# zongh5a/MDF-Net

Measured on AMD Instinct MI355X. Metric: views/sec at DTU 1600x1200x5-view x4-scale, higher is better.
Workload: dtype f32; 1 GPU; DTU eval 1600x1184 (1600x1200 cropped as load/dtueval.py:34), 5 views, 3 cost-volume stages + x2 refine = 4 output scales, hypotheses (48,24,8), batch 1 per rank, seeded random weights (pth/dtu_29.pth is not available offline); parallelism=views sharded over 1 rank(s), no collective

## Files before the change

### mdf-net_amd/csrc/conv_lds.hip

```cpp
#include <cstdlib>
#include <mutex>
#include <type_traits>
#include "common.h"

#include "conv_lds_common.h"

namespace {

constexpr int kSchedSlots = 128;
__device__ unsigned g_sched[2 * kSchedSlots];
#ifdef MDF_STAMPS
__device__ unsigned long long g_stamps[8];
#define STAMP() __builtin_readcyclecounter()
#endif

template <typename C, int KD, int KHW, int SHW, int COUT, int MTL, int ST = 0>
__device__ __forceinline__ void step(const float* const (&planes)[KD], __amdgpu_buffer_rsrc_t wres, int wvoff, const LdsConvParams& p,
                                     size_t row_vox, int w0, int q, int n16, const float (&wr)[C::WN][C::NT][C::KPL],
                                     const float (&al)[C::NT][4], const float (&be)[C::NT][4], const float (&wfirst)[2][C::NT][C::KPL]) {
  constexpr int NT = C::NT;
  extern __shared__ __attribute__((aligned(16))) float lds_base_[];
  const float* epi_tab = lds_base_ + C::EPI_OFF;
  static_assert(ST == 0 || COUT % 4 == 0, "epilogue sums need Cout % 4 == 0");
  f32x4 acc[MTL][NT];
// ... 681 lines not shown
    long long ipb = C::STREAM ? 2 : ((C::RD == 2 && blocks_per_cu == 1) ? 3 : 6);
    if (const char* e = getenv("MDF_CONV_ITEMS_PER_BLOCK")) { if (atoi(e) > 0) ipb = atoi(e); }
    long long want = (ipb * max_grid + tiles - 1) / tiles;
    if (want < 1) want = 1;
    if (want > p.D / 3) want = p.D / 3;
    if (want < 1) want = 1;
    int dch = (int)((p.D + want - 1) / want);
    if (C::RD == 2 && (dch & 1)) ++dch;
    {
      const long long items0 = tiles * ((p.D + dch - 1) / dch);
      if (items0 > max_grid && items0 < 3 * (long long)max_grid) {
        const long long rounds0 = (items0 + max_grid - 1) / max_grid;
        for (int d2 = dch + C::RD; d2 <= p.D + C::RD - 1; d2 += C::RD) {
          if (tiles * ((p.D + d2 - 1) / d2) <= max_grid) {
            if (10 * (d2 + C::NPL - 1) < 9 * rounds0 * (dch + C::NPL - 1)) dch = d2;
            break;
          }
        }
      }
    }
    if (const char* e = getenv("MDF_CONV_DCH")) { if (atoi(e) > 0) dch = atoi(e); }
    if (C::RD == 2 && (dch & 1)) ++dch;
    p.dch = dch;
    p.dchunks = (p.D + dch - 1) / dch;
    const long long items = tiles * p.dchunks;
    if (items > 0x7fffffff) return mdf::fail(MDF_EARG, "conv_lds: too many work items");
    p.n_items = (int)items;
  } else {
    if (p.D != 1) return mdf::fail(MDF_EARG, "2-D conv path needs D == 1");
    if (tiles > 0x7fffffff) return mdf::fail(MDF_EARG, "conv_lds: too many tiles");
    p.n_tiles = (int)tiles;
    p.tiles_per_item = 0;
    long long tpb = 2;
    if (const char* e = getenv("MDF_CONV2D_TILES_PER_BLOCK")) { if (atoi(e) > 0) tpb = atoi(e); }
    long long g = tiles / tpb;
    if (g < 256) g = 256;
    if (g > max_grid) g = max_grid;
    if (g > tiles) g = tiles;
    p.n_items = (int)g;
    p.dch = 1; p.dchunks = 1;
  }
  static bool attr_done_dev[64] = {};
  int dev_id = 0;
  (void)hipGetDevice(&dev_id);
  bool& attr_done = attr_done_dev[(dev_id >= 0 && dev_id < 64) ? dev_id : 0];
  if (!attr_done || dev_id >= 64) {
    hipError_t e = hipFuncSetAttribute(reinterpret_cast<const void*>(&conv_lds_kernel<CIN, CIN_MEM, COUT, KD, KHW, SHW, MT, RW, WG, ST>),
                                       hipFuncAttributeMaxDynamicSharedMemorySize, (int)kLds);
    if (e != hipSuccess) return mdf::fail(MDF_EHIP, "hipFuncSetAttribute(dynamic LDS %zu): %s", kLds, hipGetErrorString(e));
    attr_done = true;
  }
  int grid = max_grid;
  if (const char* g = getenv("MDF_CONV_GRID")) { if (atoi(g) > 0) grid = atoi(g); }
  if (grid > p.n_items) grid = p.n_items;
  if (ST) {
    if (KD == 1) {
      const int G = p.stat_groups > 0 ? p.stat_groups : 1;
      int bpg = grid / G;
      if (bpg < 1) bpg = 1;
      grid = G * bpg;
      p.stat_slices = mdf::conv_stat_slices(bpg, p.stat_slices);
    } else {
      p.stat_slices = mdf::conv_stat_slices(grid, p.stat_slices);
    }
  }
  if (getenv("MDF_CONV_DEBUG")) {
    int nb = -1;
    hipError_t e = hipOccupancyMaxActiveBlocksPerMultiprocessor(&nb, conv_lds_kernel<CIN, CIN_MEM, COUT, KD, KHW, SHW, MT, RW, WG, ST>, 256, kLds);
    hipFuncAttributes fa{};
    (void)hipFuncGetAttributes(&fa, reinterpret_cast<const void*>(&conv_lds_kernel<CIN, CIN_MEM, COUT, KD, KHW, SHW, MT, RW, WG, ST>));
    fprintf(stderr, "[conv_lds<%d,%d,%d,%d,%d,%d,%d,rw%d>] LDS %zu B dyn + %zu static, regs %d, occupancy API: %d blocks/CU (%s), grid %d, items %d\n",
            CIN, CIN_MEM, COUT, KD, KHW, SHW, MT, RW, kLds, fa.sharedSizeBytes, fa.numRegs, nb, hipGetErrorString(e), grid, p.n_items);
  }
  hipLaunchKernelGGL((conv_lds_kernel<CIN, CIN_MEM, COUT, KD, KHW, SHW, MT, RW, WG, ST>), dim3(grid), dim3(256), kLds, st, p);
  return mdf::check_launch("conv_lds_kernel");
}

}

#ifdef MDF_STAMPS
extern "C" int mdf_debug_read_stamps(unsigned long long* out8, int reset) {
  hipError_t e = hipMemcpyFromSymbol(out8, HIP_SYMBOL(g_stamps), sizeof(unsigned long long) * 8);
  if (e != hipSuccess) return -3;
  if (reset) {
    unsigned long long z[8] = {0};
    (void)hipMemcpyToSymbol(HIP_SYMBOL(g_stamps), z, sizeof z);
  }
  return 0;
}
#endif

#define LDS_CASE(ci, cim, co, kd, k, s, mt)                                                      \
  if (!stat && Cin == ci && Cin_mem == cim && Cout == co && KD == kd && KHW == k && stride == s) \
    return launch_lds<ci, cim, co, kd, k, s, mt>(p, (hipStream_t)stream);
#define LDS_CASE_T(ci, cim, co, kd, k, s, mt)                                                    \
  if (Cin == ci && Cin_mem == cim && Cout == co && KD == kd && KHW == k && stride == s)          \
    return !stat ? launch_lds<ci, cim, co, kd, k, s, mt>(p, (hipStream_t)stream) : (stat->mode == 1 ? launch_lds<ci, cim, co, kd, k, s, mt, 1, 0, 1>(p, (hipStream_t)stream) : launch_lds<ci, cim, co, kd, k, s, mt, 1, 0, 2>(p, (hipStream_t)stream));

namespace {
std::mutex g_slot_mu;
void* g_slot_stream[kSchedSlots];
bool g_slot_used[kSchedSlots];
}

static int sched_slot_of(void* stream) {
  std::lock_guard<std::mutex> lock(g_slot_mu);
  int free_slot = -1;
  for (int i = 0; i < kSchedSlots; ++i) {
    if (g_slot_used[i] && g_slot_stream[i] == stream) return i;
    if (!g_slot_used[i] && free_slot < 0) free_slot = i;
  }
  if (free_slot >= 0) { g_slot_used[free_slot] = true; g_slot_stream[free_slot] = stream; }
  return free_slot;
}

extern "C" int mdf_release_stream(void* stream) {
  std::lock_guard<std::mutex> lock(g_slot_mu);
  for (int i = 0; i < kSchedSlots; ++i)
    if (g_slot_used[i] && g_slot_stream[i] == stream) { g_slot_used[i] = false; g_slot_stream[i] = nullptr; return MDF_OK; }
  return MDF_OK;
}

#define LDS_CASE_RW(ci, cim, co, kd, k, s, mt, rw)                                               \
  if (!stat && use_rw && Cin == ci && Cin_mem == cim && Cout == co && KD == kd && KHW == k && stride == s && !res_up) { \
    p.wpack = wpack + (size_t)kd * k * k * ci * 16;                                              \
    return launch_lds<ci, cim, co, kd, k, s, mt, rw>(p, (hipStream_t)stream);                    \
  }
#define LDS_CASE_RW_T(ci, cim, co, kd, k, s, mt, rw)                                             \
  if (use_rw && Cin == ci && Cin_mem == cim && Cout == co && KD == kd && KHW == k && stride == s && !res_up) { \
    p.wpack = wpack + (size_t)kd * k * k * ci * 16;                                              \
    return !stat ? launch_lds<ci, cim, co, kd, k, s, mt, rw>(p, (hipStream_t)stream) : (stat->mode == 1 ? launch_lds<ci, cim, co, kd, k, s, mt, rw, 0, 1>(p, (hipStream_t)stream) : launch_lds<ci, cim, co, kd, k, s, mt, rw, 0, 2>(p, (hipStream_t)stream)); \
  }

#define LDS_CASE_WG(ci, co)                                                                      \
  if (use_wg && KD == 3 && KHW == 3 && stride == 1 && Cin == ci && Cin_mem == ci && Cout == co && !res_up) { \
    p.wpack = wpack + (size_t)27 * ci * (((co + 15) / 16) * 16) + (co == 8 ? (size_t)36 * ci * 16 : 0); \
    return !stat ? launch_lds<ci, ci, co, 3, 3, 1, 1, 2, 1>(p, (hipStream_t)stream) : (stat->mode == 1 ? launch_lds<ci, ci, co, 3, 3, 1, 1, 2, 1, 1>(p, (hipStream_t)stream) : launch_lds<ci, ci, co, 3, 3, 1, 1, 2, 1, 2>(p, (hipStream_t)stream)); \
  }
#define LDS_CASE_WG2(ci, co)                                                                     \
  if (use_wg && KD == 1 && KHW == 3 && stride == 1 && Cin == ci && Cin_mem == ci && Cout == co && !res_up && (!shuffle2 || (ci == 16 && co == 32) || (ci == 32 && co == 64))) { \
    p.wpack = wpack + (size_t)9 * ci * (((co + 15) / 16) * 16);                                  \
    return !stat ? launch_lds<ci, ci, co, 1, 3, 1, 1, 2, 1>(p, (hipStream_t)stream) : (stat->mode == 1 ? launch_lds<ci, ci, co, 1, 3, 1, 1, 2, 1, 1>(p, (hipStream_t)stream) : launch_lds<ci, ci, co, 1, 3, 1, 1, 2, 1, 2>(p, (hipStream_t)stream)); \
  }

#define LDS_CASE_WD(ci)                                                                          \
  if (use_wd && KD == 3 && KHW == 3 && stride == 1 && Cin == ci && Cin_mem == ci && Cout == 8 && !res_up && D >= 2) { \
    p.wpack = wpack + (size_t)27 * ci * 16 + (size_t)36 * ci * 16 + (ci == 16 ? (size_t)3 * 16 * 64 * 4 : 0); \
    if (ci == 16 && wd_stream && !stat) return launch_lds<ci, ci, 8, 3, 3, 1, 1, 2, 3>(p, (hipStream_t)stream); \
    return !stat ? launch_lds<ci, ci, 8, 3, 3, 1, 1, 2, 2>(p, (hipStream_t)stream) : (stat->mode == 1 ? launch_lds<ci, ci, 8, 3, 3, 1, 1, 2, 2, 1>(p, (hipStream_t)stream) : launch_lds<ci, ci, 8, 3, 3, 1, 1, 2, 2, 2>(p, (hipStream_t)stream)); \
  }

int mdf_wino3d_dispatch(const float* x, const float* wpack_wino, const float* alpha, const float* beta, const float* res, float res_scale,
                        float* y, int B, int D, int H, int W, int Cin, int Cout, int relu, void* stream);
int mdf_wino2d_dispatch(const float* x, const float* wpack_wino, const float* alpha, const float* beta, const float* res, float res_scale,
                        float* y, int B, int H, int W, int Cin, int Cout, int relu, void* stream);
int mdf_wino2d_s2d_dispatch(const float* x, const float* wpack_k5w, const float* alpha, const float* beta, float* y, int B, int Ho, int Wo,
                            int Cin_mem, int Cout, int relu, void* stream);

int mdf_conv_lds_dispatch(const float* x, const float* wpack, const float* alpha, const float* beta, const float* res,
                          float res_scale, const float* res_up, float* y, int B, int D, int H, int W, int Cin, int Cin_mem, int Cout, int KD,
                          int KHW, int stride, int relu, void* stream, int planar_in, int shuffle2, const mdf::ConvStat* stat) {
  static const int wd_mask = [] { const char* e = getenv("MDF_CONV_WD"); return e ? atoi(e) : 3; }();
  const bool wd_stream = [] { const char* e = getenv("MDF_CONV_WD_STREAM"); return e ? atoi(e) != 0 : true; }();
  static const bool use_wg = [] { const char* e = getenv("MDF_CONV_WINOGRAD"); return e ? atoi(e) != 0 : true; }();
  static const bool use_rw = [] { const char* e = getenv("MDF_CONV_RW"); return e ? atoi(e) != 0 : true; }();
  LdsConvParams p{};
  p.x = x; p.wpack = wpack; p.alpha = alpha; p.beta = beta; p.res = res; p.res_scale = res_scale; p.res_up = res_up; p.y = y;
  p.B = B; p.D = D; p.H = H; p.W = W; p.relu = relu; p.planar_in = planar_in; p.shuffle2 = shuffle2;
  if (stat) {
    if (Cout % 4 != 0 || shuffle2 || res_up) return mdf::fail(MDF_EUNSUPPORTED, "epilogue sums: Cout %% 4 == 0, no pixel-shuffle / upsample-add");
    p.stat_mode = stat->mode; p.stat_y = stat->y; p.stat_aux = stat->aux; p.stat_out = stat->out; p.stat_slices = stat->nslices;
    p.stat_groups = (KD == 1 && stat->group_imgs > 0) ? B / stat->group_imgs : 1;
  }
  p.sched_slot = sched_slot_of(stream);
  if (p.sched_slot < 0) return mdf::fail(MDF_EUNSUPPORTED, "conv kernels support up to %d distinct HIP streams per process", kSchedSlots);
  {
    const char* e = getenv("MDF_CONV_PREFETCH_EARLY");
    p.prefetch_early = e ? atoi(e) : 0;
  }
  const int pad = (KHW - 1) / 2;
  p.Ho = (H + 2 * pad - KHW) / stride + 1;
  p.Wo = (W + 2 * pad - KHW) / stride + 1;
  {
    const bool k5w = [] { const char* e = getenv("MDF_CONV_K5_WINOGRAD"); return e ? atoi(e) != 0 : true; }();
    if (use_wg && k5w && KD == 1 && KHW == 5 && stride == 2 && !stat && !res_up && !shuffle2 && !planar_in && H % 2 == 0 && W % 2 == 0) {
      const bool use_w2 = [] { const char* e = getenv("MDF_CONV_WINO2D"); return e ? atoi(e) != 0 : true; }();
      if (use_w2 && !res && Cin == Cin_mem && ((Cin == 16 && Cout == 32) || (Cin == 8 && Cout == 16))) {
        const size_t plain = (size_t)25 * 64 * (Cin == 16 ? 2 * 4 : 1 * 2);
        const int rc = mdf_wino2d_s2d_dispatch(x, wpack + plain, alpha, beta, y, B, p.Ho, p.Wo, Cin, Cout, relu, stream);
        if (rc != MDF_EUNSUPPORTED) return rc;
      }
      if (Cin == 16 && Cin_mem == 16 && Cout == 32) {
        p.s2d = 1; p.wpack = wpack + (size_t)25 * 1 * 2 * 64 * 4;
        return launch_lds<64, 64, 32, 1, 3, 1, 1, 2, 1>(p, (hipStream_t)stream);
      }
    }
  }
  if (shuffle2 && Cout == 64 && !use_wg) return mdf::fail(MDF_EUNSUPPORTED, "pixel-shuffle store for Cout = 64 is built into the Winograd form only (MDF_CONV_WINOGRAD=0 is set)");
  { const bool use_wd = use_wg && (wd_mask & 1); LDS_CASE_WD(8) }
  { const bool use_wd = use_wg && (wd_mask & 2); LDS_CASE_WD(16) }
  {
    const bool use_w3 = [] { const char* e = getenv("MDF_CONV_WINO3D"); return e ? atoi(e) != 0 : true; }();
    if (use_wg && use_w3 && !stat && KD == 3 && KHW == 3 && stride == 1 && Cin == Cin_mem && !res_up && !shuffle2 && Cout % 16 == 0) {
      const int rc = mdf_wino3d_dispatch(x, wpack + (size_t)27 * Cin * Cout, alpha, beta, res, res_scale, y, B, D, H, W, Cin, Cout, relu, stream);
      if (rc != MDF_EUNSUPPORTED) return rc;
    }
  }
  {
    const bool use_w2 = [] { const char* e = getenv("MDF_CONV_WINO2D"); return e ? atoi(e) != 0 : true; }();
    if (use_wg && use_w2 && !stat && KD == 1 && KHW == 3 && stride == 1 && Cin == Cin_mem && !res_up && !shuffle2 && !planar_in && D == 1) {
      const int rc = mdf_wino2d_dispatch(x, wpack + (size_t)9 * Cin * (((Cout + 15) / 16) * 16), alpha, beta, res, res_scale, y, B, H, W, Cin, Cout, relu, stream);
      if (rc != MDF_EUNSUPPORTED) return rc;
    }
  }
  LDS_CASE_WG(16, 16) LDS_CASE_WG(32, 16) LDS_CASE_WG(32, 32) LDS_CASE_WG(16, 8) LDS_CASE_WG(16, 32)
  LDS_CASE_WG2(16, 16) LDS_CASE_WG2(32, 32) LDS_CASE_WG2(64, 64) LDS_CASE_WG2(16, 32) LDS_CASE_WG2(32, 64)
  LDS_CASE_RW_T(16, 16, 8, 3, 3, 1, 2, 2) LDS_CASE_RW_T(8, 8, 8, 3, 3, 1, 2, 2)
  LDS_CASE_RW(16, 16, 4, 1, 3, 1, 1, 4) LDS_CASE_RW(8, 8, 4, 1, 3, 1, 1, 4)
  LDS_CASE_RW_T(8, 8, 8, 1, 3, 1, 2, 2) LDS_CASE_RW_T(4, 3, 8, 1, 3, 1, 2, 2) LDS_CASE_RW(4, 1, 8, 1, 3, 1, 2, 2)
  LDS_CASE(32, 32, 16, 3, 3, 1, 2) LDS_CASE(16, 16, 16, 3, 3, 1, 4) LDS_CASE(16, 16, 8, 3, 3, 1, 4) LDS_CASE(8, 8, 8, 3, 3, 1, 4)
  LDS_CASE(32, 32, 32, 3, 3, 1, 2)
  LDS_CASE(16, 16, 32, 3, 3, 1, 2) LDS_CASE(8, 8, 16, 3, 3, 1, 4)
  LDS_CASE(4, 3, 8, 1, 3, 1, 4) LDS_CASE(8, 8, 8, 1, 3, 1, 4) LDS_CASE(16, 16, 16, 1, 3, 1, 4) LDS_CASE(32, 32, 32, 1, 3, 1, 2)
  LDS_CASE(64, 64, 64, 1, 3, 1, 1)
  LDS_CASE_T(8, 8, 16, 1, 5, 2, 2) LDS_CASE_T(16, 16, 32, 1, 5, 2, 2) LDS_CASE_T(32, 32, 64, 1, 5, 2, 1)
  LDS_CASE(16, 16, 32, 1, 1, 1, 4)
  LDS_CASE(16, 16, 64, 1, 1, 1, 4) LDS_CASE(32, 32, 64, 1, 1, 1, 2) LDS_CASE(64, 64, 16, 1, 1, 1, 1) LDS_CASE(64, 64, 32, 1, 1, 1, 1)
  LDS_CASE(64, 64, 64, 1, 1, 1, 1)
  LDS_CASE(32, 32, 32, 1, 1, 1, 2) LDS_CASE(32, 32, 16, 1, 1, 1, 2) LDS_CASE(16, 16, 16, 1, 1, 1, 4)
  LDS_CASE(4, 1, 8, 1, 3, 1, 4) LDS_CASE(8, 8, 32, 1, 3, 1, 4) LDS_CASE(8, 8, 1, 1, 3, 1, 4)
  LDS_CASE(32, 32, 8, 1, 3, 1, 2)
  LDS_CASE(16, 16, 32, 1, 3, 1, 2) LDS_CASE(32, 32, 64, 1, 3, 1, 1)
  LDS_CASE(16, 16, 4, 1, 3, 1, 4) LDS_CASE(8, 8, 4, 1, 3, 1, 4)
  return MDF_EUNSUPPORTED;
}
```

### mdf-net_amd/csrc/wino3d.hip

```cpp
#include <cstdlib>
#include <type_traits>
#include "common.h"
#include "conv_lds_common.h"
#include "wino3d_acc.h"

namespace {

template <int I, int N, typename F>
__device__ __forceinline__ void static_for(F&& f) {
  if constexpr (I < N) {
    f(std::integral_constant<int, I>{});
    static_for<I + 1, N>(f);
  }
}

struct Wino3dParams {
  const float* x;
  const float* wpack;
  const float* alpha;
  const float* beta;
  const float* res;
  float* y;
  float res_scale;
  int B, D, H, W, relu;
// ... 207 lines not shown
          float ov[4];
#pragma unroll
          for (int k = 0; k < 4; ++k) {
            ov[k] = yv[pr][rr][k] * al_l[k] + be_l[k];
            if (p.relu) ov[k] = fmaxf(ov[k], 0.f);
          }
          const size_t oi = (row_vox + ow) * COUT + c0;
          if (p.res) {
            const float4 rv = *reinterpret_cast<const float4*>(p.res + oi);
            ov[0] = rv.x + ov[0] * p.res_scale; ov[1] = rv.y + ov[1] * p.res_scale;
            ov[2] = rv.z + ov[2] * p.res_scale; ov[3] = rv.w + ov[3] * p.res_scale;
          }
          if (!(MDF_W3_DIAG & 2) || ov[0] == 1234.5f) *reinterpret_cast<float4*>(p.y + oi) = make_float4(ov[0], ov[1], ov[2], ov[3]);
        }
      }
    };

    auto step = [&](auto rc, int zi, int z_next2, bool has_next, bool k0, bool k1, bool k2, bool fresh1) {
      constexpr int R = decltype(rc)::value;
      const bool all3 = MDF_W3_NOMASK || (k0 && k1 && k2 && !fresh1);
      if (MDF_W3_PF_AT_START) issue_plane(has_next ? zi + 1 : -1);
      constexpr int SLOT_N = (R + 1) % 3;
      static_for<0, NSTEP>([&](auto ic) {
        constexpr int i = decltype(ic)::value;
        constexpr int ch = i / 16, ab = i % 16;
        constexpr bool last_chunk = (ch == NCH - 1);
        if (!(MDF_W3_DIAG & 16)) load_a((i + AH) % NSTEP, (i + AH) % NA);
        if constexpr (ch == 0 && ab == WRITE_AB) {
          if (has_next) {
            write_plane(SLOT_N);
            __syncthreads();
          }
        }
        if constexpr (ab > WRITE_AB && ab <= WRITE_AB + 8) {
          constexpr int e0 = 2 * (ab - WRITE_AB - 1);
          if constexpr (!last_chunk) { read_elem(R, ch + 1, e0); read_elem(R, ch + 1, e0 + 1); }
          else { read_elem(SLOT_N, 0, e0); read_elem(SLOT_N, 0, e0 + 1); }
        }
        __builtin_amdgcn_sched_barrier(0);
        constexpr int S0 = ((R + 1) % 3) * 16 + ab, S1 = R * 16 + ab, S2 = ((R + 2) % 3) * 16 + ab;
        if (__builtin_expect(all3, 1)) {
          if constexpr (ch == 0) AccTile<S0>::mfma_fresh(af[i % NA][0][0], V[ab][0][0]);
          else AccTile<S0>::mfma(af[i % NA][0][0], V[ab][0][0]);
          AccTile<S0>::mfma(af[i % NA][0][1], V[ab][0][1]);
          AccTile<S0>::mfma(af[i % NA][0][2], V[ab][1][0]);
          AccTile<S0>::mfma(af[i % NA][0][3], V[ab][1][1]);
          AccTile<S1>::mfma(af[i % NA][1][0], V[ab][0][0]);
          AccTile<S1>::mfma(af[i % NA][1][1], V[ab][0][1]);
          AccTile<S1>::mfma(af[i % NA][1][2], V[ab][1][0]);
          AccTile<S1>::mfma(af[i % NA][1][3], V[ab][1][1]);
          AccTile<S2>::mfma(af[i % NA][2][0], V[ab][0][0]);
          AccTile<S2>::mfma(af[i % NA][2][1], V[ab][0][1]);
          AccTile<S2>::mfma(af[i % NA][2][2], V[ab][1][0]);
          AccTile<S2>::mfma(af[i % NA][2][3], V[ab][1][1]);
        } else {
          if (k0) {
            if constexpr (ch == 0) AccTile<S0>::mfma_fresh(af[i % NA][0][0], V[ab][0][0]);
            else AccTile<S0>::mfma(af[i % NA][0][0], V[ab][0][0]);
            AccTile<S0>::mfma(af[i % NA][0][1], V[ab][0][1]);
            AccTile<S0>::mfma(af[i % NA][0][2], V[ab][1][0]);
            AccTile<S0>::mfma(af[i % NA][0][3], V[ab][1][1]);
          }
          if (k1) {
            if constexpr (ch == 0) {
              if (fresh1) AccTile<S1>::mfma_fresh(af[i % NA][1][0], V[ab][0][0]);
              else AccTile<S1>::mfma(af[i % NA][1][0], V[ab][0][0]);
            } else {
              AccTile<S1>::mfma(af[i % NA][1][0], V[ab][0][0]);
            }
            AccTile<S1>::mfma(af[i % NA][1][1], V[ab][0][1]);
            AccTile<S1>::mfma(af[i % NA][1][2], V[ab][1][0]);
            AccTile<S1>::mfma(af[i % NA][1][3], V[ab][1][1]);
          }
          if (k2) {
            AccTile<S2>::mfma(af[i % NA][2][0], V[ab][0][0]);
            AccTile<S2>::mfma(af[i % NA][2][1], V[ab][0][1]);
            AccTile<S2>::mfma(af[i % NA][2][2], V[ab][1][0]);
            AccTile<S2>::mfma(af[i % NA][2][3], V[ab][1][1]);
          }
        }
        __builtin_amdgcn_sched_barrier(0);
        if constexpr (ab == 15 && !last_chunk) { if (!(MDF_W3_DIAG & 8)) transform(); }
      });
      if (!MDF_W3_PF_AT_START) issue_plane(z_next2);
      if (!(MDF_W3_DIAG & 8)) transform();
      if (k2 && !(MDF_W3_DIAG & 4)) epilogue(std::integral_constant<int, (R + 2) % 3>{}, zi - 1);
    };

    int zi = (da == 0) ? 0 : da - 1;
    const int z_last = (db == p.D) ? p.D - 1 : db;
    __syncthreads();
    issue_plane(zi);
    write_plane(0);
    __syncthreads();
    if (!MDF_W3_PF_AT_START) issue_plane(zi < z_last ? zi + 1 : -1);
#pragma unroll
    for (int e = 0; e < 16; ++e) read_elem(0, 0, e);
    transform();
#pragma unroll
    for (int i = 0; i < AH; ++i) load_a(i, i % NA);

    int r_last = 0;
#define W3_STEP(RR)                                                                                          \
    {                                                                                                        \
      const bool has_next = zi < z_last;                                                                     \
      step(std::integral_constant<int, RR>{}, zi, (zi + 2 <= z_last) ? zi + 2 : -1, has_next,                \
           zi + 1 >= da && zi + 1 < db, zi >= da && zi < db, zi - 1 >= da && zi - 1 < db, zi == 0);          \
      if (!has_next) { r_last = RR; break; }                                                                 \
      ++zi;                                                                                                  \
    }
    for (;;) {
      W3_STEP(0)
      W3_STEP(1)
      W3_STEP(2)
    }
#undef W3_STEP
    if (db == p.D) {
      switch (r_last) {
        case 0: epilogue(std::integral_constant<int, 0>{}, p.D - 1); break;
        case 1: epilogue(std::integral_constant<int, 1>{}, p.D - 1); break;
        default: epilogue(std::integral_constant<int, 2>{}, p.D - 1); break;
      }
    }
  }
}

template <int CIN, int COUT>
int launch_wino3d(Wino3dParams& p, hipStream_t st) {
  typedef W3<CIN, COUT> C;
  constexpr int NA = MDF_W3_NA;
  constexpr int WRITE_AB = MDF_W3_WRITE_AB;
  p.tiles_h = (p.H + C::TH - 1) / C::TH;
  p.tiles_w = (p.W + C::TWO - 1) / C::TWO;
  p.total = (long long)p.B * p.tiles_h * p.tiles_w * p.D;
  if (p.total >= (1ll << 31)) return MDF_EUNSUPPORTED;
  auto kern = &wino3d_kernel<CIN, COUT, NA, WRITE_AB>;
  static bool attr_done_dev[64] = {};
  int dev_id = 0;
  (void)hipGetDevice(&dev_id);
  bool& attr_done = attr_done_dev[(dev_id >= 0 && dev_id < 64) ? dev_id : 0];
  if (!attr_done || dev_id >= 64) {
    hipError_t e = hipFuncSetAttribute(reinterpret_cast<const void*>(kern), hipFuncAttributeMaxDynamicSharedMemorySize, (int)C::LDS_BYTES);
    if (e != hipSuccess) return mdf::fail(MDF_EHIP, "hipFuncSetAttribute(dynamic LDS %zu): %s", (size_t)C::LDS_BYTES, hipGetErrorString(e));
    attr_done = true;
  }
  long long grid = 256;
  if (const char* g = getenv("MDF_WINO3D_GRID")) { if (atoi(g) > 0) grid = atoi(g); }
  if (grid > p.total / 4) grid = p.total / 4;
  if (grid < 1) grid = 1;
  hipLaunchKernelGGL(kern, dim3((unsigned)grid), dim3(256), C::LDS_BYTES, st, p);
  return mdf::check_launch("wino3d_kernel");
}

}

int mdf_wino3d_dispatch(const float* x, const float* wpack_wino, const float* alpha, const float* beta, const float* res, float res_scale,
                        float* y, int B, int D, int H, int W, int Cin, int Cout, int relu, void* stream) {
  Wino3dParams p{};
  p.x = x; p.wpack = wpack_wino; p.alpha = alpha; p.beta = beta; p.res = res; p.res_scale = res_scale; p.y = y;
  p.B = B; p.D = D; p.H = H; p.W = W; p.relu = relu;
  if ((long long)H * W * Cin * 4 >= (1ll << 31)) return MDF_EUNSUPPORTED;
  if (Cin == 32 && Cout == 16) return launch_wino3d<32, 16>(p, (hipStream_t)stream);
  if (Cin == 16 && Cout == 16) return launch_wino3d<16, 16>(p, (hipStream_t)stream);
  return MDF_EUNSUPPORTED;
}
```

### mdf-net_amd/mdfnet_hip/kernel_families.py

```python
import re

MFMA_CONV = "mfma_conv"
WARP = "warp_aggregate"
WARP_TRAIN = "aggregate_train_passes"
WARP_SCATTER = "aggregate_scatter"
WGRAD = "wgrad"
BN = "batchnorm_train"
PROB = "prob_head"
HEADS = "heads"
FILTER = "consistency_filter"
POINT_EVAL = "point_eval"
CONTROL = "control"

KERNEL_FAMILY = {
    "conv_lds_kernel": MFMA_CONV, "conv3d_kernel": MFMA_CONV, "conv3d_wlds_kernel": MFMA_CONV, "convtr_all_kernel": MFMA_CONV, "convtr_cls_kernel": MFMA_CONV, "conv_pair_kernel": MFMA_CONV, "conv_pair_valu_kernel": MFMA_CONV,
    "conv1x1_kernel": MFMA_CONV, "conv1x1_heads_kernel": MFMA_CONV, "refine_tail_kernel": MFMA_CONV, "prob_fused_kernel": MFMA_CONV, "res_pair_kernel": MFMA_CONV,
    "wino3d_kernel": MFMA_CONV, "wino2d_kernel": MFMA_CONV,
    "pack_weights_kernel": CONTROL, "pack_batch_kernel": CONTROL,
    "warp_kernel": WARP, "warp_vec8_kernel": WARP, "warp_vec_win_kernel": WARP, "corner_index_kernel": WARP,
    "warp_train_kernel": WARP_TRAIN, "warp_bwd_kernel": WARP_SCATTER,
    "agg_prepare_kernel": CONTROL, "agg_finalize_kernel": CONTROL, "agg_bwd_finalize_kernel": WARP_SCATTER,
    "wgrad_kernel": WGRAD, "wgrad_a1_kernel": WGRAD, "wgrad_a1_valu_kernel": WGRAD, "wgrad2d_kernel": WGRAD,
    "wgrad_lds_kernel": WGRAD, "wgrad_lds_batch_kernel": WGRAD, "slab_sum_kernel": WGRAD, "slab_sum_batch_kernel": WGRAD,
    "bn_reduce_kernel": BN, "bn_finalize_kernel": BN, "bn_relu_apply_kernel": BN, "bn_finalize_apply_kernel": BN,
    "bn_relu_bwd_kernel": BN,
    "prob_head_kernel": PROB, "prob_head_tiled_kernel": PROB, "prob_from_partials_kernel": PROB,
    "softmax_regress_bwd_kernel": PROB, "prob_conv_dgrad_kernel": PROB, "upsample2_bwd_kernel": PROB,
    "depth_regress_kernel": HEADS, "confidence_kernel": HEADS, "confidence_up2_kernel": HEADS, "range_affine_kernel": HEADS,
    "hypos_fit_kernel": HEADS, "hypos_from_fit_kernel": HEADS, "refine_head_kernel": HEADS, "fpn_compose_fwd_kernel": HEADS, "fpn_compose_bwd_kernel": HEADS,
    "consistency_fuse_kernel": FILTER,
    "consensus_fuse_kernel": FILTER, "consensus_scan_kernel": FILTER, "consensus_compact_kernel": FILTER,
    "pcd_reproj_kernel": FILTER, "pcd_cand_count_kernel": FILTER, "pcd_cand_place_kernel": FILTER, "pcd_select_kernel": FILTER, "pcd_select_big_kernel": FILTER, "pcd_bin_sum_kernel": FILTER, "pcd_bin_offsets_kernel": FILTER,
    "pcd_seg_init_kernel": FILTER, "pcd_seg_hook_kernel": FILTER, "pcd_seg_count_kernel": FILTER, "pcd_seg_apply_kernel": FILTER,
    "pcd_count_kernel": FILTER, "pcd_scan_kernel": FILTER, "pcd_compact_kernel": FILTER,
    "pts_bbox_kernel": POINT_EVAL, "pts_bbox_final_kernel": POINT_EVAL, "pts_morton_kernel": POINT_EVAL, "pts_sort_hist_kernel": POINT_EVAL,
    "pts_sort_scan_kernel": POINT_EVAL, "pts_sort_scatter_kernel": POINT_EVAL, "pts_gather_kernel": POINT_EVAL, "pts_leaf_kernel": POINT_EVAL,
    "pts_node_kernel": POINT_EVAL, "pts_nn_kernel": POINT_EVAL, "pts_rank_kernel": POINT_EVAL, "pts_radius_kernel": POINT_EVAL,
    "pts_reduce_init_kernel": POINT_EVAL, "pts_reduce_round_kernel": POINT_EVAL, "pts_reduce_step_kernel": POINT_EVAL,
    "pts_reduce_keep_kernel": POINT_EVAL, "pts_dtu_masks_kernel": POINT_EVAL,
    "masked_smooth_l1_reduce_kernel": CONTROL, "masked_smooth_l1_finalize_kernel": CONTROL, "masked_smooth_l1_bwd_kernel": CONTROL,
    "masked_smooth_l1_reduce_multi_kernel": CONTROL, "masked_smooth_l1_bwd_multi_kernel": CONTROL, "adam_step_kernel": CONTROL,
}

def function_name(rocprof_name):
    s = rocprof_name.strip()
    if s.startswith("void "):
        s = s[5:]
    s = s.replace("(anonymous namespace)::", "")
    head = re.split(r"[<(]", s, maxsplit=1)[0]
    return head.split("::")[-1].strip()


def family(rocprof_name):
    return KERNEL_FAMILY.get(function_name(rocprof_name))


def is_ours(rocprof_name):
    return function_name(rocprof_name) in KERNEL_FAMILY


def globals_in_sources(csrc_dir):
    import os
    names = {}
    for f in sorted(os.listdir(csrc_dir)):
        if not f.endswith(".hip"):
            continue
        text = open(os.path.join(csrc_dir, f)).read()
        for m in re.finditer(r"__global__\b[\s\S]*?\bvoid\s+([A-Za-z_][A-Za-z_0-9]*)\s*\(", text):
            names.setdefault(m.group(1), f)
    return names


def fetch_size_factor(rocprof_name):
    return 2.0
```

Before: 279.1 views/s.

## Add Winograd 3D pair kernel for Cout=8 depth-pair conv3d

Adds a new wino3d_pair_kernel that computes 3x3x3 convolutions with Cin 8 or 16 and Cout 8, two output depth planes per pass. It uses an F(2x2,3x3) Winograd transform in H and W with MFMA accumulation over a 4-slot LDS plane ring, and streams depth planes so that each input plane feeds two output planes. The dispatcher routes these convs to the new kernel before the existing LDS direct-conv WD path, which remains the fallback. The new kernel has a large LDS footprint and a complex software pipeline, which risks lower occupancy and subtle indexing bugs.

```diff
diff --git a/mdf-net_amd/csrc/conv_lds.hip b/mdf-net_amd/csrc/conv_lds.hip
--- a/mdf-net_amd/csrc/conv_lds.hip
+++ b/mdf-net_amd/csrc/conv_lds.hip
@@ -857,6 +857,8 @@
 
 int mdf_wino3d_dispatch(const float* x, const float* wpack_wino, const float* alpha, const float* beta, const float* res, float res_scale,
                         float* y, int B, int D, int H, int W, int Cin, int Cout, int relu, void* stream);
+int mdf_wino3d_pair_dispatch(const float* x, const float* wpack_wd, const float* alpha, const float* beta, const float* res, float res_scale,
+                             float* y, int B, int D, int H, int W, int Cin, int relu, void* stream);
 int mdf_wino2d_dispatch(const float* x, const float* wpack_wino, const float* alpha, const float* beta, const float* res, float res_scale,
                         float* y, int B, int H, int W, int Cin, int Cout, int relu, void* stream);
 int mdf_wino2d_s2d_dispatch(const float* x, const float* wpack_k5w, const float* alpha, const float* beta, float* y, int B, int Ho, int Wo,
@@ -902,6 +904,15 @@
     }
   }
   if (shuffle2 && Cout == 64 && !use_wg) return mdf::fail(MDF_EUNSUPPORTED, "pixel-shuffle store for Cout = 64 is built into the Winograd form only (MDF_CONV_WINOGRAD=0 is set)");
+  {
+    const bool use_w3 = [] { const char* e = getenv("MDF_CONV_WINO3D"); return e ? atoi(e) != 0 : true; }();
+    const bool use_wd = use_wg && (Cin == 8 ? (wd_mask & 1) : Cin == 16 ? (wd_mask & 2) : 0);
+    if (use_wd && use_w3 && !stat && !res_up && !shuffle2 && KD == 3 && KHW == 3 && stride == 1 && Cin == Cin_mem && Cout == 8 && D >= 2) {
+      const size_t off = (size_t)27 * Cin * 16 + (size_t)36 * Cin * 16 + (Cin == 16 ? (size_t)3 * 16 * 64 * 4 : 0);
+      const int rc = mdf_wino3d_pair_dispatch(x, wpack + off, alpha, beta, res, res_scale, y, B, D, H, W, Cin, relu, stream);
+      if (rc != MDF_EUNSUPPORTED) return rc;
+    }
+  }
   { const bool use_wd = use_wg && (wd_mask & 1); LDS_CASE_WD(8) }
   { const bool use_wd = use_wg && (wd_mask & 2); LDS_CASE_WD(16) }
   {
diff --git a/mdf-net_amd/csrc/wino3d.hip b/mdf-net_amd/csrc/wino3d.hip
--- a/mdf-net_amd/csrc/wino3d.hip
+++ b/mdf-net_amd/csrc/wino3d.hip
@@ -383,6 +383,323 @@
   return mdf::check_launch("wino3d_kernel");
 }
 
+template <int CIN>
+struct W3P {
+  static_assert(CIN == 8 || CIN == 16, "pair form: Cin 8 or 16 (one chunk of 4 lanes x KPL channels)");
+  static constexpr int KPL = CIN / 4, NV = KPL / 2;
+  static constexpr int TH = 8, TWO = 32;
+  static constexpr int PH = TH + 2, PW = TWO + 2, NPP = PH * PW;
+  static constexpr int S = round_s(NPP, KPL, 2);
+  static constexpr int PLANE = CIN * S;
+  static constexpr int RING = 4;
+  static constexpr int NPOS = 4 * NPP;
+  static constexpr int NFILL = (NPOS + 255) / 256;
+  static constexpr int FRAG = 64 * KPL;
+  static constexpr int W_OFF = RING * PLANE;
+  static constexpr size_t LDS_BYTES = (size_t)(W_OFF + 4 * 16 * FRAG) * sizeof(float);
+  static_assert(LDS_BYTES <= 160 * 1024, "LDS");
+  static_assert(S > NPP, "a pad vector per group takes the fill's surplus lanes");
+  static_assert(PLANE % 4 == 0, "16-B aligned slots and fragments");
+};
+
+template <int T, bool FRESH, int KPL>
+__device__ __forceinline__ void pair_mfma(const float (&a)[KPL], const f32x2_t (&v)[KPL / 2]) {
+  if constexpr (FRESH) AccTile<T>::mfma_fresh(a[0], v[0][0]);
+  else AccTile<T>::mfma(a[0], v[0][0]);
+  AccTile<T>::mfma(a[1], v[0][1]);
+  if constexpr (KPL == 4) {
+    AccTile<T>::mfma(a[2], v[1][0]);
+    AccTile<T>::mfma(a[3], v[1][1]);
+  }
+}
+
+template <int CIN, int NA, int WRITE_AB>
+__global__ __launch_bounds__(256, 1) void wino3d_pair_kernel(const Wino3dParams p) {
+  typedef W3P<CIN> C;
+  constexpr int KPL = C::KPL, NV = C::NV, S = C::S, PW = C::PW, NPP = C::NPP, NFILL = C::NFILL;
+  constexpr int AH = NA - 1, NSTEP = 16;
+  static_assert(NSTEP % NA == 0, "the fragment ring must close over a plane");
+  typedef typename VecT<KPL>::type vec_t;
+  extern __shared__ __attribute__((aligned(16))) float lds[];
+
+  const int tid = threadIdx.x, lane = tid & 63;
+  const int wm = __builtin_amdgcn_readfirstlane(tid >> 6);
+  const int q = lane >> 4, n16 = lane & 15;
+  const int lane_lds = (q * S + wm * 2 * PW + n16 * 2) * KPL;
+  float al_l[4], be_l[4];
+#pragma unroll
+  for (int k = 0; k < 4; ++k) {
+    const int c = ((4 * q) & 7) + k;
+    al_l[k] = p.alpha ? p.alpha[c] : 1.f;
+    be_l[k] = p.beta ? p.beta[c] : 0.f;
+  }
+  for (int v = tid; v < 4 * 16 * C::FRAG / 4; v += 256)
+    *reinterpret_cast<float4*>(lds + C::W_OFF + v * 4) = *reinterpret_cast<const float4*>(p.wpack + (size_t)v * 4);
+
+  int f_lds[NFILL];
+#pragma unroll
+  for (int k = 0; k < NFILL; ++k) {
+    const int idx = tid + k * 256;
+    f_lds[k] = (idx < C::NPOS) ? ((idx & 3) * S + (idx >> 2)) * KPL : NPP * KPL;
+  }
+  const size_t plane_elems = (size_t)p.H * p.W * CIN;
+  const unsigned plane_bytes = (unsigned)(plane_elems * 4);
+  const int NP = (p.D + 1) >> 1;
+
+  const unsigned lb = mdf::xcd_remap(blockIdx.x, gridDim.x);
+  unsigned s_cur = (unsigned)((unsigned long long)lb * (unsigned)p.total / gridDim.x);
+  const unsigned s_end = (unsigned)((unsigned long long)(lb + 1) * (unsigned)p.total / gridDim.x);
+
+  while (s_cur < s_end) {
+    const int tile_l = __builtin_amdgcn_readfirstlane((int)(s_cur / (unsigned)NP));
+    const int pa = __builtin_amdgcn_readfirstlane((int)(s_cur - (unsigned)tile_l * (unsigned)NP));
+    const int pb = __builtin_amdgcn_readfirstlane((int)min((unsigned)NP, (unsigned)pa + (s_end - s_cur)));
+    s_cur += pb - pa;
+    const int tw = __builtin_amdgcn_readfirstlane(tile_l % p.tiles_w);
+    const int th = __builtin_amdgcn_readfirstlane((tile_l / p.tiles_w) % p.tiles_h);
+    const int b = __builtin_amdgcn_readfirstlane(tile_l / (p.tiles_w * p.tiles_h));
+    const int h0 = th * C::TH, w0 = tw * C::TWO;
+    const bool wave_live = (h0 + 2 * wm) < p.H;
+
+    unsigned f_off[NFILL];
+    {
+      int tid_l = tid;
+      asm volatile("" : "+v"(tid_l));
+#pragma unroll
+      for (int k = 0; k < NFILL; ++k) {
+        const int idx = tid_l + k * 256;
+        const int v = idx >> 2;
+        const int ih = h0 - 1 + v / PW, iw = w0 - 1 + v % PW;
+        const bool ok = idx < C::NPOS && ih >= 0 && ih < p.H && iw >= 0 && iw < p.W;
+        f_off[k] = ok ? (unsigned)(((ih * p.W + iw) * CIN + (idx & 3) * KPL) * 4) : 0x80000000u;
+      }
+    }
+    const float* xb = p.x + (size_t)b * p.D * plane_elems;
+    vec_t pf[NFILL];
+    auto issue_plane = [&](int z) {
+      const bool in = z >= 0 && z < p.D;
+      const unsigned long long pa64 = (unsigned long long)(xb + (size_t)(in ? z : 0) * plane_elems);
+      const unsigned lo = (unsigned)__builtin_amdgcn_readfirstlane((int)(unsigned)pa64), hi = (unsigned)__builtin_amdgcn_readfirstlane((int)(unsigned)(pa64 >> 32));
+      const unsigned nrec = (MDF_W3_DIAG & 1) ? 0u : (unsigned)__builtin_amdgcn_readfirstlane((int)(in ? plane_bytes : 0u));
+      const __amdgpu_buffer_rsrc_t xr = make_rsrc((const void*)(((unsigned long long)hi << 32) | lo), nrec);
+#pragma unroll
+      for (int k = 0; k < NFILL; ++k) {
+        if constexpr (KPL == 4) {
+          const u32x4_t v = __builtin_amdgcn_raw_buffer_load_b128(xr, (int)f_off[k], 0, 0);
+          pf[k] = make_float4(__uint_as_float(v.x), __uint_as_float(v.y), __uint_as_float(v.z), __uint_as_float(v.w));
+        } else {
+          const u32x2_t v = __builtin_amdgcn_raw_buffer_load_b64(xr, (int)f_off[k], 0, 0);
+          pf[k] = make_float2(__uint_as_float(v.x), __uint_as_float(v.y));
+        }
+      }
+    };
+    auto write_plane = [&](int slot) {
+#pragma unroll
+      for (int k = 0; k < NFILL; ++k) *reinterpret_cast<vec_t*>(lds + slot * C::PLANE + f_lds[k]) = pf[k];
+    };
+
+    f32x2_t V[16][NV];
+    f32x2_t Dn[16][NV];
+    auto read_elem = [&](int slot, int e) {
+      const int i = e >> 2, j = e & 3;
+      float t[KPL];
+      lds_frag<KPL>(lds + slot * C::PLANE + lane_lds + (i * PW + j) * KPL, t);
+#pragma unroll
+      for (int c = 0; c < NV; ++c) Dn[e][c] = (f32x2_t){t[2 * c], t[2 * c + 1]};
+    };
+    auto transform = [&]() {
+#pragma unroll
+      for (int j = 0; j < 4; ++j)
+#pragma unroll
+        for (int c = 0; c < NV; ++c) {
+          const f32x2_t d0 = Dn[j][c], d1 = Dn[4 + j][c], d2 = Dn[8 + j][c], d3 = Dn[12 + j][c];
+          Dn[j][c] = d0 - d2; Dn[4 + j][c] = d1 + d2; Dn[8 + j][c] = d2 - d1; Dn[12 + j][c] = d1 - d3;
+        }
+#pragma unroll
+      for (int a = 0; a < 4; ++a)
+#pragma unroll
+        for (int c = 0; c < NV; ++c) {
+          const f32x2_t e0 = Dn[a * 4][c], e1 = Dn[a * 4 + 1][c], e2 = Dn[a * 4 + 2][c], e3 = Dn[a * 4 + 3][c];
+          V[a * 4][c] = e0 - e2; V[a * 4 + 1][c] = e1 + e2; V[a * 4 + 2][c] = e2 - e1; V[a * 4 + 3][c] = e1 - e3;
+        }
+#pragma unroll
+      for (int e = 0; e < 16; ++e)
+#pragma unroll
+        for (int c = 0; c < NV; ++c) asm volatile("" : "+v"(V[e][c]));
+    };
+
+    float af[NA][2][KPL];
+    auto load_a = [&](int i, int buf, int jl) {
+      lds_frag<KPL>(lds + C::W_OFF + (jl * NSTEP + i) * C::FRAG + lane * KPL, af[buf][0]);
+      lds_frag<KPL>(lds + C::W_OFF + ((jl + 2) * NSTEP + i) * C::FRAG + lane * KPL, af[buf][1]);
+    };
+
+    auto epilogue = [&](auto setc, int pr) {
+      constexpr int SET = decltype(setc)::value;
+      if (!wave_live) return;
+      const int o = 2 * pr + (q >> 1), c0 = (4 * q) & 7;
+      asm volatile("s_nop 15\n\ts_nop 15" ::: "memory");
+      float yv[2][2][4];
+      static_for<0, 2>([&](auto k2c) {
+        constexpr int k2 = decltype(k2c)::value;
+        float m[16][2];
+        static_for<0, 16>([&](auto abc) { AccTile<SET * 16 + decltype(abc)::value>::template read2<k2>(m[decltype(abc)::value]); });
+        f32x2_t srow[2][4];
+#pragma unroll
+        for (int bb = 0; bb < 4; ++bb) {
+          const f32x2_t m0 = {m[bb][0], m[bb][1]}, m1 = {m[4 + bb][0], m[4 + bb][1]};
+          const f32x2_t m2 = {m[8 + bb][0], m[8 + bb][1]}, m3 = {m[12 + bb][0], m[12 + bb][1]};
+          srow[0][bb] = m0 + m1 + m2;
+          srow[1][bb] = m1 - m2 - m3;
+        }
+#pragma unroll
+        for (int r = 0; r < 2; ++r) {
+          const f32x2_t y0 = srow[r][0] + srow[r][1] + srow[r][2];
+          const f32x2_t y1 = srow[r][1] - srow[r][2] - srow[r][3];
+          yv[r][0][2 * k2] = y0[0]; yv[r][0][2 * k2 + 1] = y0[1];
+          yv[r][1][2 * k2] = y1[0]; yv[r][1][2 * k2 + 1] = y1[1];
+        }
+      });
+      if (o >= p.D) return;
+#pragma unroll
+      for (int r = 0; r < 2; ++r) {
+        const int h = h0 + 2 * wm + r;
+        if (h >= p.H) continue;
+        const size_t row_vox = (((size_t)b * p.D + o) * p.H + h) * p.W;
+#pragma unroll
+        for (int rr = 0; rr < 2; ++rr) {
+          const int ow = w0 + 2 * n16 + rr;
+          if (ow >= p.W) continue;
+          float ov[4];
+#pragma unroll
+          for (int k = 0; k < 4; ++k) {
+            ov[k] = yv[r][rr][k] * al_l[k] + be_l[k];
+            if (p.relu) ov[k] = fmaxf(ov[k], 0.f);
+          }
+          const size_t oi = (row_vox + ow) * 8 + c0;
+          if (p.res) {
+            const float4 rv = *reinterpret_cast<const float4*>(p.res + oi);
+            ov[0] = rv.x + ov[0] * p.res_scale; ov[1] = rv.y + ov[1] * p.res_scale;
+            ov[2] = rv.z + ov[2] * p.res_scale; ov[3] = rv.w + ov[3] * p.res_scale;
+          }
+          if (!(MDF_W3_DIAG & 2) || ov[0] == 1234.5f) *reinterpret_cast<float4*>(p.y + oi) = make_float4(ov[0], ov[1], ov[2], ov[3]);
+        }
+      }
+    };
+
+    auto step = [&](auto rc, auto firstc, int zi, int z_next2, bool has_next, bool kl, bool ke, int pl) {
+      constexpr int R = decltype(rc)::value;
+      constexpr bool FIRST = decltype(firstc)::value;
+      constexpr int L = (R < 2) ? 0 : 1, E = 1 - L;
+      constexpr int JL = R & 1, JLN = (R + 1) & 1;
+      constexpr int SLOT_N = (R + 1) % 4;
+      constexpr bool FRESH_L = FIRST || JL == 0;
+      const bool both = kl && ke;
+      static_for<0, NSTEP>([&](auto ic) {
+        constexpr int ab = decltype(ic)::value;
+        if constexpr (MDF_W3_DIAG & 16) {
+        } else if constexpr (ab + AH < NSTEP) load_a(ab + AH, (ab + AH) % NA, JL);
+        else load_a(ab + AH - NSTEP, (ab + AH) % NA, JLN);
+        if constexpr (ab == WRITE_AB) {
+          if (has_next) {
+            write_plane(SLOT_N);
+            __syncthreads();
+          }
+        }
+        if constexpr (ab > WRITE_AB && ab <= WRITE_AB + 8) {
+          constexpr int e0 = 2 * (ab - WRITE_AB - 1);
+          read_elem(SLOT_N, e0); read_elem(SLOT_N, e0 + 1);
+        }
+        __builtin_amdgcn_sched_barrier(0);
+        constexpr int TL = L * 16 + ab, TE = E * 16 + ab;
+        if constexpr (FIRST) {
+          pair_mfma<TL, true, KPL>(af[ab % NA][0], V[ab]);
+        } else if (__builtin_expect(both, 1)) {
+          pair_mfma<TL, FRESH_L, KPL>(af[ab % NA][0], V[ab]);
+          pair_mfma<TE, false, KPL>(af[ab % NA][1], V[ab]);
+        } else {
+          if (kl) pair_mfma<TL, FRESH_L, KPL>(af[ab % NA][0], V[ab]);
+          if (ke) pair_mfma<TE, false, KPL>(af[ab % NA][1], V[ab]);
+        }
+        __builtin_amdgcn_sched_barrier(0);
+      });
+      issue_plane(z_next2);
+      if (!(MDF_W3_DIAG & 8)) transform();
+      if constexpr ((R & 1) && !FIRST) { if (ke && !(MDF_W3_DIAG & 4)) epilogue(std::integral_constant<int, E>{}, pl - 1); }
+    };
+
+    const int z0 = (pa == 0) ? 0 : 2 * pa - 1;
+    const int z_last = min(2 * pb, p.D - 1);
+    const bool peel = (pa == 0);
+    const int slot0 = peel ? 3 : 0;
+    __syncthreads();
+    issue_plane(z0);
+    write_plane(slot0);
+    __syncthreads();
+    issue_plane(z0 < z_last ? z0 + 1 : -1);
+#pragma unroll
+    for (int e = 0; e < 16; ++e) read_elem(slot0, e);
+    transform();
+#pragma unroll
+    for (int i = 0; i < AH; ++i) load_a(i, i % NA, peel ? 1 : 0);
+
+    int zi = z0, r_last = 3;
+    bool more = true;
+    if (peel) {
+      more = zi < z_last;
+      step(std::integral_constant<int, 3>{}, std::true_type{}, zi, (zi + 2 <= z_last) ? zi + 2 : -1, more, true, false, (zi + 1) >> 1);
+      ++zi;
+    }
+#define W3P_STEP(RR)                                                                                         \
+    {                                                                                                        \
+      const bool has_next = zi < z_last;                                                                     \
+      const int pl = (zi + 1) >> 1;                                                                          \
+      step(std::integral_constant<int, RR>{}, std::false_type{}, zi, (zi + 2 <= z_last) ? zi + 2 : -1, has_next, \
+           pl >= pa && pl < pb, pl - 1 >= pa && pl - 1 < pb, pl);                                             \
+      if (!has_next) { r_last = RR; break; }                                                                 \
+      ++zi;                                                                                                  \
+    }
+    if (more) {
+      for (;;) {
+        W3P_STEP(0)
+        W3P_STEP(1)
+        W3P_STEP(2)
+        W3P_STEP(3)
+      }
+    }
+#undef W3P_STEP
+    if (pb == NP && !(MDF_W3_DIAG & 4)) {
+      if (r_last == 0 || r_last == 3) epilogue(std::integral_constant<int, 1>{}, NP - 1);
+      else epilogue(std::integral_constant<int, 0>{}, NP - 1);
+    }
+  }
+}
+
+template <int CIN>
+int launch_wino3d_pair(Wino3dParams& p, hipStream_t st) {
+  typedef W3P<CIN> C;
+  p.tiles_h = (p.H + C::TH - 1) / C::TH;
+  p.tiles_w = (p.W + C::TWO - 1) / C::TWO;
+  p.total = (long long)p.B * p.tiles_h * p.tiles_w * ((p.D + 1) / 2);
+  if (p.total >= (1ll << 31)) return MDF_EUNSUPPORTED;
+  auto kern = &wino3d_pair_kernel<CIN, MDF_W3_NA, MDF_W3_WRITE_AB>;
+  static bool attr_done_dev[64] = {};
+  int dev_id = 0;
+  (void)hipGetDevice(&dev_id);
+  bool& attr_done = attr_done_dev[(dev_id >= 0 && dev_id < 64) ? dev_id : 0];
+  if (!attr_done || dev_id >= 64) {
+    hipError_t e = hipFuncSetAttribute(reinterpret_cast<const void*>(kern), hipFuncAttributeMaxDynamicSharedMemorySize, (int)C::LDS_BYTES);
+    if (e != hipSuccess) return mdf::fail(MDF_EHIP, "hipFuncSetAttribute(dynamic LDS %zu): %s", (size_t)C::LDS_BYTES, hipGetErrorString(e));
+    attr_done = true;
+  }
+  long long grid = 256;
+  if (const char* g = getenv("MDF_WINO3D_GRID")) { if (atoi(g) > 0) grid = atoi(g); }
+  if (grid > p.total / 2) grid = p.total / 2;
+  if (grid < 1) grid = 1;
+  hipLaunchKernelGGL(kern, dim3((unsigned)grid), dim3(256), C::LDS_BYTES, st, p);
+  return mdf::check_launch("wino3d_pair_kernel");
+}
+
 }
 
 int mdf_wino3d_dispatch(const float* x, const float* wpack_wino, const float* alpha, const float* beta, const float* res, float res_scale,
@@ -395,3 +712,14 @@
   if (Cin == 16 && Cout == 16) return launch_wino3d<16, 16>(p, (hipStream_t)stream);
   return MDF_EUNSUPPORTED;
 }
+
+int mdf_wino3d_pair_dispatch(const float* x, const float* wpack_wd, const float* alpha, const float* beta, const float* res, float res_scale,
+                             float* y, int B, int D, int H, int W, int Cin, int relu, void* stream) {
+  Wino3dParams p{};
+  p.x = x; p.wpack = wpack_wd; p.alpha = alpha; p.beta = beta; p.res = res; p.res_scale = res_scale; p.y = y;
+  p.B = B; p.D = D; p.H = H; p.W = W; p.relu = relu;
+  if (D < 2 || (long long)H * W * Cin * 4 >= (1ll << 31)) return MDF_EUNSUPPORTED;
+  if (Cin == 16) return launch_wino3d_pair<16>(p, (hipStream_t)stream);
+  if (Cin == 8) return launch_wino3d_pair<8>(p, (hipStream_t)stream);
+  return MDF_EUNSUPPORTED;
+}
diff --git a/mdf-net_amd/mdfnet_hip/kernel_families.py b/mdf-net_amd/mdfnet_hip/kernel_families.py
--- a/mdf-net_amd/mdfnet_hip/kernel_families.py
+++ b/mdf-net_amd/mdfnet_hip/kernel_families.py
@@ -15,7 +15,7 @@
 KERNEL_FAMILY = {
     "conv_lds_kernel": MFMA_CONV, "conv3d_kernel": MFMA_CONV, "conv3d_wlds_kernel": MFMA_CONV, "convtr_all_kernel": MFMA_CONV, "convtr_cls_kernel": MFMA_CONV, "conv_pair_kernel": MFMA_CONV, "conv_pair_valu_kernel": MFMA_CONV,
     "conv1x1_kernel": MFMA_CONV, "conv1x1_heads_kernel": MFMA_CONV, "refine_tail_kernel": MFMA_CONV, "prob_fused_kernel": MFMA_CONV, "res_pair_kernel": MFMA_CONV,
-    "wino3d_kernel": MFMA_CONV, "wino2d_kernel": MFMA_CONV,
+    "wino3d_kernel": MFMA_CONV, "wino3d_pair_kernel": MFMA_CONV, "wino2d_kernel": MFMA_CONV,
     "pack_weights_kernel": CONTROL, "pack_batch_kernel": CONTROL,
     "warp_kernel": WARP, "warp_vec8_kernel": WARP, "warp_vec_win_kernel": WARP, "corner_index_kernel": WARP,
     "warp_train_kernel": WARP_TRAIN, "warp_bwd_kernel": WARP_SCATTER,
```

Result: no change. 278.5 views/s (median of 2 runs) (-0.2%).
